# ablab/spades

Measured on NVIDIA H100. Metric: Mk-mers/s (extract+count+index) k=55, 150 bp reads, higher is better.
Workload: dtype u64

## Files before the change

### spades_b200/csrc/count.cu

```cuda
#include <time.h>

#include <algorithm>
#include <chrono>
#include <memory>

#include "sgpu_internal.h"

namespace sg {

__device__ __forceinline__ void prefetch_l2(const void *p) { asm volatile("prefetch.global.L2 [%0];" ::"l"(p)); }

struct ReadsSrc {
    const uint64_t *words;
    const uint64_t *offs;
    const uint32_t *lens;
    int64_t n;
    uint64_t nwords;
    int K;
    static constexpr int kIds = 24;
    static constexpr int kIdLines = 48;
    static constexpr bool kSubRanges = true;
    __device__ __forceinline__ uint64_t first_word(int64_t item) const { return offs[item]; }
    __device__ __forceinline__ uint32_t len(int64_t item) const { return lens[item]; }
    __device__ __forceinline__ void prefetch_items(int64_t item, int lane) const {
// ... 25 lines not shown
        reinterpret_cast<ulonglong2 *>(dst)[1] = make_ulonglong2(k.w[2], k.w[3]);
    } else {
#pragma unroll
        for (int q = 0; q < NW; ++q) dst[q] = k.w[q];
    }
}
template <int NW>
__device__ __forceinline__ Kmer<NW> load_rec(const uint64_t *src) {
    Kmer<NW> k;
    if (NW == 2) {
        ulonglong2 v = *reinterpret_cast<const ulonglong2 *>(src);
        k.w[0] = v.x; k.w[1] = v.y;
    } else if (NW == 4) {
        ulonglong2 a = reinterpret_cast<const ulonglong2 *>(src)[0], b = reinterpret_cast<const ulonglong2 *>(src)[1];
        k.w[0] = a.x; k.w[1] = a.y; k.w[2] = b.x; k.w[3] = b.y;
    } else {
#pragma unroll
        for (int q = 0; q < NW; ++q) k.w[q] = src[q];
    }
    return k;
}

struct LevelA {
    int K;
    uint32_t B;
    uint32_t b_lo, b_hi;
    int rA;
    uint32_t PA;
};

template <int NW>
__device__ __forceinline__ void store_rec_stream(uint64_t *dst, const Kmer<NW> &k) {
    if (NW == 2) {
        asm volatile("st.global.L1::no_allocate.v2.u64 [%0], {%1, %2};" ::"l"(dst), "l"(k.w[0]), "l"(k.w[1]) : "memory");
    } else if (NW == 4) {
        asm volatile("st.global.L1::no_allocate.v2.u64 [%0], {%1, %2};" ::"l"(dst), "l"(k.w[0]), "l"(k.w[1]) : "memory");
        asm volatile("st.global.L1::no_allocate.v2.u64 [%0], {%1, %2};" ::"l"(dst + 2), "l"(k.w[2]), "l"(k.w[3]) : "memory");
    } else {
#pragma unroll
        for (int q = 0; q < NW; ++q) asm volatile("st.global.L1::no_allocate.u64 [%0], %1;" ::"l"(dst + q), "l"(k.w[q]) : "memory");
    }
}

__device__ __forceinline__ int find_item_u(const uint32_t *pref, int nitems, uint32_t i, uint32_t uniform) {
    if (uniform) return (int)(i / uniform);
    int lo = 0, hi = nitems - 1;
    while (lo < hi) {
        int mid = (lo + hi + 1) >> 1;
        if (pref[mid] <= i) lo = mid; else hi = mid - 1;
    }
    return lo;
}

template <int NW>
__device__ __forceinline__ bool part_of(const LevelA &p, const Kmer<NW> &k, uint32_t *part) {
    uint32_t b = kmer_bucket<NW>(k, p.B);
    if (b < p.b_lo || b >= p.b_hi) return false;
    *part = ((b - p.b_lo) << p.rA) | key_top_bits<NW>(k, p.K, p.rA);
    return true;
}

__global__ void levelA_totals_k(const uint32_t *__restrict__ blk_counts, uint32_t PA, int G, uint64_t *__restrict__ part_total) {
    uint32_t part = blockIdx.x * blockDim.x + threadIdx.x;
    if (part >= PA) return;
    uint64_t s = 0;
    for (int g = 0; g < G; ++g) s += blk_counts[(size_t)g * PA + part];
    part_total[part] = s;
}
__global__ void levelA_bases_k(const uint32_t *__restrict__ blk_counts, uint32_t stride, uint32_t PA, int G,
                               const uint64_t *__restrict__ part_start, uint64_t *__restrict__ base) {
    uint32_t part = blockIdx.x * blockDim.x + threadIdx.x;
    if (part >= PA) return;
    uint64_t run = part_start[part];
    for (int g = 0; g < G; ++g) {
        base[(size_t)g * PA + part] = run;
        run += blk_counts[(size_t)g * stride + part];
    }
}

static const int kRollC = 24;
template <bool BOTH> constexpr int kRollWin = BOTH ? kRollC / 2 : kRollC;
static_assert(kRollC <= 33 && kRollC % 8 == 0, "roll_init fetches a chunk's bases from two words; an id row is a whole number of 16-byte words");
static_assert(ReadsSrc::kIds == kRollC && KmerSetSrc::kIds % 8 == 0, "an id row holds a chunk's records");
static const int kRollThreads = 512;

static const int kRollTile = 32;
static const int kRollWarps = kRollThreads / 32;
static const int kRollStageWords = 320;
struct RollWarp {
    uint64_t words[kRollStageWords];
    uint32_t pref[kRollTile + 1];
    uint32_t len[kRollTile];
    uint32_t off[kRollTile];
    uint32_t pad_;
};
static_assert(sizeof(RollWarp) % 8 == 0, "per-warp slices stay 8-byte aligned");
static size_t roll_smem_bytes(uint32_t nslots) { return (((size_t)nslots * 4 + 15) & ~(size_t)15) + (size_t)kRollWarps * sizeof(RollWarp); }
__device__ __forceinline__ RollWarp *roll_warp_slice(unsigned char *raw, uint32_t nslots) {
    return reinterpret_cast<RollWarp *>(raw + (((size_t)nslots * 4 + 15) & ~(size_t)15)) + (threadIdx.x >> 5);
}

template <bool BOTH, class Src>
__device__ __forceinline__ uint32_t roll_warp_setup(const Src &src, int64_t item0, int nitems, RollWarp &rw, uint32_t *uniform, bool *staged) {
    const int lane = threadIdx.x & 31;
    uint32_t c = 0, L = 0;
    uint64_t a = 0, b = 0;
    if (lane < nitems) {
        L = src.len(item0 + lane);
        a = src.first_word(item0 + lane);
        b = a + (((uint64_t)L + 31) >> 5);
        const uint32_t w = (int)L >= src.K ? (uint32_t)((int)L - src.K + 1) : 0u;
        c = (w + kRollWin<BOTH> - 1) / kRollWin<BOTH>;
    }
    uint32_t inc = c;
#pragma unroll
    for (int o = 1; o < 32; o <<= 1) {
        const uint32_t t = __shfl_up_sync(0xffffffffu, inc, o);
        if (lane >= o) inc += t;
    }
    rw.len[lane] = L;
    rw.pref[lane] = inc - c;
    const uint32_t total = __shfl_sync(0xffffffffu, inc, 31);
    if (lane == 31) rw.pref[kRollTile] = total;
    const uint32_t c0 = __shfl_sync(0xffffffffu, c, 0);
    const bool same = __all_sync(0xffffffffu, lane >= nitems || c == c0);
    *uniform = (same && c0) ? c0 : 0u;
    const uint64_t w0 = __shfl_sync(0xffffffffu, a, 0);
    const bool ok = lane >= nitems || (a >= w0 && b >= a && b - w0 <= (uint64_t)kRollStageWords);
    const bool st = __all_sync(0xffffffffu, ok);
    if (st) {
        rw.off[lane] = (uint32_t)(a - w0);
        uint32_t end = lane < nitems ? (uint32_t)(b - w0) : 0u;
#pragma unroll
        for (int o = 16; o; o >>= 1) end = max(end, __shfl_xor_sync(0xffffffffu, end, o));
        uint64_t tmp[kRollStageWords / 32];
#pragma unroll
        for (int j = 0; j < kRollStageWords / 32; ++j) tmp[j] = (uint32_t)(lane + 32 * j) < end ? __ldg(src.words + w0 + lane + 32 * j) : 0ull;
#pragma unroll
        for (int j = 0; j < kRollStageWords / 32; ++j) if ((uint32_t)(lane + 32 * j) < end) rw.words[lane + 32 * j] = tmp[j];
    }
    *staged = st;
    __syncwarp();
    return total;
}

template <bool BOTH, class Src>
__global__ void roll_tile_ids_k(Src src, int64_t ntiles, uint32_t *__restrict__ out) {
    const int64_t t = (int64_t)blockIdx.x * (blockDim.x >> 5) + (threadIdx.x >> 5);
    if (t >= ntiles) return;
    const int lane = threadIdx.x & 31;
    const int64_t item = t * kRollTile + lane;
    uint32_t s = 0;
    if (item < src.n) {
        const int L = (int)src.len(item);
        const uint32_t w = L >= src.K ? (uint32_t)(L - src.K + 1) : 0u;
        s = (w + kRollWin<BOTH> - 1) / kRollWin<BOTH>;
    }
    for (int o = 16; o; o >>= 1) s += __shfl_down_sync(0xffffffffu, s, o);
    if (lane == 0) out[t] = s * Src::kIds;
}

struct RollUnit { int it, j0, cnt; };
template <bool BOTH>
__device__ __forceinline__ RollUnit roll_unit(const RollWarp &rw, int nitems, uint32_t u, uint32_t unif, int K) {
    constexpr int C = kRollWin<BOTH>;
    RollUnit q;
    q.it = find_item_u(rw.pref, nitems, u, unif);
    q.j0 = (int)(u - rw.pref[q.it]) * C;
    const int nwin = (int)rw.len[q.it] - K + 1;
    q.cnt = nwin - q.j0 < C ? nwin - q.j0 : C;
    return q;
}

template <int NW, class Src, bool BOTH>
__global__ void __launch_bounds__(kRollThreads, 2) levelA_count_roll_k(Src src, LevelA p, uint32_t *__restrict__ blk_counts,
                                                                      const uint64_t *__restrict__ tile_off, uint16_t *__restrict__ ids) {
    extern __shared__ __align__(16) unsigned char sm_raw[];
    uint32_t *hist = reinterpret_cast<uint32_t *>(sm_raw);
    RollWarp &rw = *roll_warp_slice(sm_raw, p.PA);
    for (uint32_t i = threadIdx.x; i < p.PA; i += blockDim.x) hist[i] = 0;
    __syncthreads();
    const int K = p.K;
    const int lane = threadIdx.x & 31, warp = threadIdx.x >> 5;
    const int64_t ntiles = (src.n + kRollTile - 1) / kRollTile;
    const int64_t per = (ntiles + gridDim.x - 1) / gridDim.x;
    const int64_t t0 = (int64_t)blockIdx.x * per, t1 = min(ntiles, t0 + per);
    for (int64_t t = t0 + warp; t < t1; t += kRollWarps) {
        const int64_t item0 = t * kRollTile;
        const int nitems = (int)min((int64_t)kRollTile, src.n - item0);
        uint32_t unif = 0;
        bool staged = false;
        const bool has_next = t + kRollWarps < t1;
        const int64_t nx = (t + kRollWarps) * kRollTile;
        uint64_t next_w0 = 0;
        if (has_next) {
            next_w0 = src.first_word(nx);
            src.prefetch_items(nx, lane);
        }
        const uint32_t nunits = roll_warp_setup<BOTH>(src, item0, nitems, rw, &unif, &staged);
        uint64_t *row = ids ? reinterpret_cast<uint64_t *>(ids + tile_off[t]) : nullptr;
        for (uint32_t u = lane; u < nunits; u += 32) {
            const RollUnit q = roll_unit<BOTH>(rw, nitems, u, unif, K);
            const uint64_t *seq = staged ? static_cast<const uint64_t *>(rw.words + rw.off[q.it]) : src.words + src.first_word(item0 + q.it);
            RollState<NW> st;
            roll_init<NW>(st, seq, q.j0, K, q.cnt);
            const int nrec = BOTH ? 2 * q.cnt : q.cnt;
#pragma unroll 1
            for (int g = 0; g < Src::kIds / 4; ++g) {
                uint64_t acc = 0;
#pragma unroll
                for (int e = 0; e < 4; ++e) {
                    const int s = 4 * g + e;
                    uint32_t id = 0xffffu;
                    if (s < nrec) {
                        if (s > 0 && !(BOTH && (e & 1))) roll_next<NW>(st, K);
                        const Kmer<NW> k = BOTH ? ((e & 1) ? st.r : st.f) : kmer_is_minimal<NW>(st.f, st.r) ? st.f : st.r;
                        uint32_t part;
                        if (part_of<NW>(p, k, &part)) { atomicAdd(&hist[part], 1u); id = part; }
                    }
                    acc |= (uint64_t)id << (16 * e);
                }
                if (row) row[(size_t)u * (Src::kIds / 4) + g] = acc;
            }
        }
        if (has_next && lane < 10 && next_w0 + 16 * lane < src.nwords) prefetch_l2(src.words + next_w0 + 16 * lane);
        __syncwarp();
    }
    __syncthreads();
    uint32_t *out = blk_counts + (size_t)blockIdx.x * p.PA;
    for (uint32_t i = threadIdx.x; i < p.PA; i += blockDim.x) out[i] += hist[i];
}

static const uint32_t kABatchMin = 1024;
static_assert(kABatchMin / kRollWarps >= 32 * 2, "a warp's share of the smallest batch holds one window of a warp step");
__host__ __device__ __forceinline__ size_t abatch_offset(uint32_t PA) {
    return ((((size_t)2 * PA * 4 + 15) & ~(size_t)15) + (size_t)kRollWarps * sizeof(RollWarp) + 15) & ~(size_t)15;
}
template <int NW, bool PLANNED>
constexpr size_t abatch_rec_bytes() { return NW * sizeof(uint64_t) + (PLANNED ? sizeof(uint16_t) : sizeof(uint32_t) + sizeof(uint16_t)); }

static const uint32_t kABatchNoTag = 0xffffffffu;
static const int kABatchPartBits = 13;
template <int NW, class Src, bool BOTH>
__global__ void __launch_bounds__(kRollThreads, 2) levelA_scatter_roll_k(Src src, LevelA p, uint64_t *__restrict__ base, uint64_t *__restrict__ out,
                                                                        uint32_t row_stride, uint32_t cap) {
    extern __shared__ __align__(16) unsigned char sm_raw[];
    __shared__ uint32_t s_fill;
    __shared__ uint32_t warp_tot[kRollWarps];
    const uint32_t PA = p.PA;
    uint32_t *cur = reinterpret_cast<uint32_t *>(sm_raw);
    uint32_t *cnt = cur + PA;
    RollWarp &rw = *roll_warp_slice(sm_raw, 2 * PA);
    uint64_t *stage = reinterpret_cast<uint64_t *>(sm_raw + abatch_offset(PA));
    uint32_t *tags = reinterpret_cast<uint32_t *>(stage + (size_t)cap * NW);
    uint16_t *idx = reinterpret_cast<uint16_t *>(tags + cap);
    uint64_t *mybase = base + (size_t)blockIdx.x * row_stride;
    const uint64_t region0 = mybase[0];
    for (uint32_t i = threadIdx.x; i < PA; i += blockDim.x) { cur[i] = (uint32_t)(mybase[i] - region0); cnt[i] = 0; }
    if (threadIdx.x == 0) s_fill = 0;
    __syncthreads();
    uint64_t *const out0 = out + region0 * NW;
    const int K = p.K;
    const int lane = threadIdx.x & 31, warp = threadIdx.x >> 5;
    const uint32_t lt_mask = (1u << lane) - 1u;
    const int64_t ntiles = (src.n + kRollTile - 1) / kRollTile;
    const int64_t per = (ntiles + gridDim.x - 1) / gridDim.x;
    const int64_t t0 = (int64_t)blockIdx.x * per, t1 = min(ntiles, t0 + per);

    int64_t t = t0 + warp;
    bool need_setup = true;
    int nitems = 0;
    uint32_t nunits = 0, unif = 0;
    bool staged = false;
    uint64_t next_w0 = 0;
    int u = 0, s = 0, cnt_w = 0;
    RollState<NW> st;
    for (;;) {
        while (t < t1) {
            if (need_setup) {
                const int64_t item0 = t * kRollTile;
                nitems = (int)min((int64_t)kRollTile, src.n - item0);
                const int64_t nx = (t + kRollWarps) * kRollTile;
                if (t + kRollWarps < t1) {
                    next_w0 = src.first_word(nx);
                    src.prefetch_items(nx, lane);
                }
                nunits = roll_warp_setup<BOTH>(src, item0, nitems, rw, &unif, &staged);
                u = lane - 32; s = cnt_w = 0;
                need_setup = false;
            }
            if (s >= cnt_w && u < (int)nunits) {
                u += 32;
                if (u < (int)nunits) {
                    const RollUnit q = roll_unit<BOTH>(rw, nitems, (uint32_t)u, unif, K);
                    const uint64_t *seq = staged ? static_cast<const uint64_t *>(rw.words + rw.off[q.it]) : src.words + src.first_word(t * kRollTile + q.it);
                    roll_init<NW>(st, seq, q.j0, K, q.cnt);
                    s = 0; cnt_w = BOTH ? 2 * q.cnt : q.cnt;
                }
            }
            const bool act = s < cnt_w;
            if (!__any_sync(0xffffffffu, act)) {
                if (t + kRollWarps < t1 && lane < 10 && next_w0 + 16 * lane < src.nwords) prefetch_l2(src.words + next_w0 + 16 * lane);
                __syncwarp();
                t += kRollWarps;
                need_setup = true;
                continue;
            }
            uint32_t part = 0;
            bool mine = false;
            Kmer<NW> k;
            if (act) {
                const bool fwd = BOTH ? !(s & 1) : kmer_is_minimal<NW>(st.f, st.r);
#pragma unroll
                for (int j = 0; j < NW; ++j) k.w[j] = fwd ? st.f.w[j] : st.r.w[j];
                mine = part_of<NW>(p, k, &part);
            }
            const uint32_t bal = __ballot_sync(0xffffffffu, mine);
            if (bal) {
                const uint32_t n = __popc(bal);
                uint32_t b0 = 0;
                if (lane == 0) b0 = atomicAdd(&s_fill, n);
                b0 = __shfl_sync(0xffffffffu, b0, 0);
                if (b0 + n > cap) {
                    if (b0 < cap && (uint32_t)lane < cap - b0) tags[b0 + lane] = kABatchNoTag;
                    break;
                }
                if (mine) {
                    const uint32_t i = b0 + __popc(bal & lt_mask);
                    const uint32_t rank = atomicAdd(&cnt[part], 1u) & 0xffffu;
                    store_rec<NW>(stage + (size_t)i * NW, k);
                    tags[i] = (rank << kABatchPartBits) | part;
                }
            }
            if (act && ++s < cnt_w && (!BOTH || !(s & 1))) roll_next<NW>(st, K);
        }
        const bool more = __syncthreads_or(t < t1);
        const uint32_t nslots = min(s_fill, cap);
        const uint32_t own = (PA + kRollThreads - 1) / kRollThreads;
        const uint32_t j0 = min(PA, threadIdx.x * own), j1 = min(PA, j0 + own);
        uint32_t sum = 0;
        for (uint32_t j = j0; j < j1; ++j) sum += cnt[j] & 0xffffu;
        uint32_t inc = sum;
#pragma unroll
        for (int o = 1; o < 32; o <<= 1) {
            const uint32_t v = __shfl_up_sync(0xffffffffu, inc, o);
            if (lane >= o) inc += v;
        }
        if (lane == 31) warp_tot[warp] = inc;
        __syncthreads();
        uint32_t wb = 0, total = 0;
#pragma unroll
        for (int w = 0; w < kRollWarps; ++w) { const uint32_t v = warp_tot[w]; if (w < warp) wb += v; total += v; }
        uint32_t o = wb + inc - sum;
        for (uint32_t j = j0; j < j1; ++j) {
            const uint32_t c = cnt[j] & 0xffffu;
            o += c;
            cnt[j] = o << 16;
            cur[j] += c;
        }
        if (threadIdx.x == 0) s_fill = 0;
        __syncthreads();
        for (uint32_t i = threadIdx.x; i < nslots; i += kRollThreads) {
            const uint32_t tg = tags[i];
            if (tg == kABatchNoTag) continue;
            idx[(cnt[tg & ((1u << kABatchPartBits) - 1)] >> 16) - 1 - (tg >> kABatchPartBits)] = (uint16_t)i;
        }
        __syncthreads();
        for (uint32_t q = threadIdx.x; q < total; q += kRollThreads) {
            const uint32_t i = idx[q], tg = tags[i];
            const uint32_t slot = cur[tg & ((1u << kABatchPartBits) - 1)] - 1 - (tg >> kABatchPartBits);
            store_rec_stream<NW>(out0 + (size_t)slot * NW, load_rec<NW>(stage + (size_t)i * NW));
        }
        __syncthreads();
        if (!more) break;
    }
    for (uint32_t i = threadIdx.x; i < PA; i += blockDim.x) mybase[i] = region0 + cur[i];
}

template <int NW, class Src, bool BOTH>
__global__ void __launch_bounds__(kRollThreads, 2) levelA_scatter_plan_k(Src src, LevelA p, uint64_t *__restrict__ base, uint64_t *__restrict__ out,
                                                                        const uint64_t *__restrict__ tile_off, const uint16_t *__restrict__ ids,
                                                                        uint32_t id_lo, uint32_t row_stride, uint32_t q_lo, uint64_t ids_len, uint32_t cap) {
    extern __shared__ __align__(16) unsigned char sm_raw[];
    __shared__ uint32_t warp_tot[kRollWarps];
    constexpr int kR = BOTH ? 2 : 1;
    constexpr int kRowV = Src::kIds / 8;
    const uint32_t PA = p.PA;
    uint32_t *cur = reinterpret_cast<uint32_t *>(sm_raw);
    uint32_t *run = cur + PA;
    RollWarp &rw = *roll_warp_slice(sm_raw, 2 * PA);
    uint64_t *stage = reinterpret_cast<uint64_t *>(sm_raw + abatch_offset(PA));
    uint16_t *ptag = reinterpret_cast<uint16_t *>(stage + (size_t)cap * NW);
    uint64_t *mybase = base + (size_t)blockIdx.x * row_stride + q_lo;
    const uint64_t region0 = mybase[0];
    for (uint32_t i = threadIdx.x; i < PA; i += blockDim.x) { cur[i] = (uint32_t)(mybase[i] - region0); run[i] = 0; }
    __syncthreads();
    uint64_t *const out0 = out + region0 * NW;
    const int K = p.K;
    const int lane = threadIdx.x & 31, warp = threadIdx.x >> 5;
    const int64_t ntiles = (src.n + kRollTile - 1) / kRollTile;
    const int64_t per = (ntiles + gridDim.x - 1) / gridDim.x;
    const int64_t t0 = (int64_t)blockIdx.x * per, t1 = min(ntiles, t0 + per);
    const uint32_t share = cap / kRollWarps;

    int64_t pt = t0 + warp;
    int pj = 0, ps = 0;
    uint32_t pn = 0;
    bool p_enter = true;
    const ulonglong2 *prow = nullptr;
    int64_t rt = pt;
    int rj = 0, rs = 0;
    bool need_setup = true;
    int nitems = 0;
    uint32_t nunits = 0, unif = 0;
    bool staged = false;
    uint64_t next_w0 = 0;
    const ulonglong2 *row = nullptr;
    for (;;) {
        uint32_t room = share;
        while (pt < t1) {
            if (p_enter) {
                const uint64_t a = tile_off[pt], b = tile_off[pt + 1];
                if (pt + kRollWarps < t1) {
                    const uint64_t nr = tile_off[pt + kRollWarps];
                    if ((Src::kIdLines >= 32 || lane < Src::kIdLines) && nr + 64 * lane < ids_len) prefetch_l2(ids + nr + 64 * lane);
                    if (lane < Src::kIdLines - 32 && nr + 64 * (32 + lane) < ids_len) prefetch_l2(ids + nr + 64 * (32 + lane));
                }
                pn = (uint32_t)((b - a) / Src::kIds);
                prow = reinterpret_cast<const ulonglong2 *>(ids + a);
                p_enter = false;
            }
            if ((uint32_t)pj * 32 >= pn) {
                pt += kRollWarps; pj = 0; ps = 0; p_enter = true;
                continue;
            }
            if (room < 32 * kR) break;
            const uint32_t u = (uint32_t)pj * 32 + lane;
            uint64_t idq[Src::kIds / 4];
#pragma unroll
            for (int v = 0; v < kRowV; ++v) {
                ulonglong2 x = make_ulonglong2(~0ull, ~0ull);
                if (u < pn) x = __ldg(prow + (size_t)u * kRowV + v);
                idq[2 * v] = x.x; idq[2 * v + 1] = x.y;
            }
            int end = Src::kIds;
#pragma unroll
            for (int e = 0; e < Src::kIds; e += kR) {
                uint32_t part[kR];
                bool own[kR];
                uint32_t c = 0;
#pragma unroll
                for (int r = 0; r < kR; ++r) {
                    part[r] = (uint32_t)((idq[(e + r) / 4] >> (16 * ((e + r) % 4))) & 0xffffu) - id_lo;
                    own[r] = e >= ps && part[r] < PA;
                    c += __popc(__ballot_sync(0xffffffffu, own[r]));
                }
                if (c > room) { end = e; break; }
                room -= c;
#pragma unroll
                for (int r = 0; r < kR; ++r) if (own[r]) atomicAdd(&run[part[r]], 1u);
            }
            if (end < Src::kIds) { ps = end; break; }
            ++pj; ps = 0;
        }
        const bool more = __syncthreads_or(pt < t1);
        const uint32_t own = (PA + kRollThreads - 1) / kRollThreads;
        const uint32_t j0 = min(PA, threadIdx.x * own), j1 = min(PA, j0 + own);
        uint32_t sum = 0;
        for (uint32_t j = j0; j < j1; ++j) sum += run[j] & 0xffffu;
        uint32_t inc = sum;
#pragma unroll
        for (int o = 1; o < 32; o <<= 1) {
            const uint32_t v = __shfl_up_sync(0xffffffffu, inc, o);
            if (lane >= o) inc += v;
        }
        if (lane == 31) warp_tot[warp] = inc;
        __syncthreads();
        uint32_t wb = 0, total = 0;
#pragma unroll
        for (int w = 0; w < kRollWarps; ++w) { const uint32_t v = warp_tot[w]; if (w < warp) wb += v; total += v; }
        uint32_t o = wb + inc - sum;
        for (uint32_t j = j0; j < j1; ++j) {
            const uint32_t c = run[j] & 0xffffu;
            run[j] = o << 16;
            o += c;
            cur[j] += c;
        }
        __syncthreads();
        while (rt < pt || (rt == pt && (rj < pj || (rj == pj && rs < ps)))) {
            if (need_setup) {
                const int64_t item0 = rt * kRollTile;
                nitems = (int)min((int64_t)kRollTile, src.n - item0);
                const int64_t nx = (rt + kRollWarps) * kRollTile;
                if (rt + kRollWarps < t1) {
                    next_w0 = src.first_word(nx);
                    src.prefetch_items(nx, lane);
                }
                nunits = roll_warp_setup<BOTH>(src, item0, nitems, rw, &unif, &staged);
                row = reinterpret_cast<const ulonglong2 *>(ids + tile_off[rt]);
                need_setup = false;
            }
            if ((uint32_t)rj * 32 >= nunits) {
                if (rt + kRollWarps < t1 && lane < 10 && next_w0 + 16 * lane < src.nwords) prefetch_l2(src.words + next_w0 + 16 * lane);
                __syncwarp();
                rt += kRollWarps; rj = 0; rs = 0;
                need_setup = true;
                continue;
            }
            const int end = (rt == pt && rj == pj) ? ps : Src::kIds;
            const int u = rj * 32 + lane;
            if (u < (int)nunits) {
                const RollUnit q = roll_unit<BOTH>(rw, nitems, (uint32_t)u, unif, K);
                const int s_end = min(end, BOTH ? 2 * q.cnt : q.cnt);
                if (rs < s_end) {
                    uint64_t idq[Src::kIds / 4];
#pragma unroll
                    for (int v = 0; v < kRowV; ++v) {
                        const ulonglong2 x = __ldg(row + (size_t)u * kRowV + v);
                        idq[2 * v] = x.x; idq[2 * v + 1] = x.y;
                    }
                    for (int w = 0; w < rs / 4; ++w) {
#pragma unroll
                        for (int v = 0; v + 1 < Src::kIds / 4; ++v) idq[v] = idq[v + 1];
                    }
                    idq[0] >>= 16 * (rs & 3);
                    const uint64_t *seq = staged ? static_cast<const uint64_t *>(rw.words + rw.off[q.it]) : src.words + src.first_word(rt * kRollTile + q.it);
                    RollState<NW> st;
                    roll_init<NW>(st, seq, q.j0 + rs / kR, K, q.cnt - rs / kR);
                    for (int s = rs;;) {
                        const uint32_t part = (uint32_t)(idq[0] & 0xffffu) - id_lo;
                        if (part < PA) {
                            const bool fwd = BOTH ? !(s & 1) : kmer_is_minimal<NW>(st.f, st.r);
                            Kmer<NW> k;
#pragma unroll
                            for (int j = 0; j < NW; ++j) k.w[j] = fwd ? st.f.w[j] : st.r.w[j];
                            const uint32_t pos = atomicAdd(&run[part], 1u << 16) >> 16;
                            store_rec<NW>(stage + (size_t)pos * NW, k);
                            ptag[pos] = (uint16_t)part;
                        }
                        if (++s >= s_end) break;
                        if (!BOTH || !(s & 1)) roll_next<NW>(st, K);
                        if ((s & 3) == 0) {
#pragma unroll
                            for (int v = 0; v + 1 < Src::kIds / 4; ++v) idq[v] = idq[v + 1];
                        } else {
                            idq[0] >>= 16;
                        }
                    }
                }
            }
            if (end == Src::kIds) { ++rj; rs = 0; } else rs = end;
        }
        __syncthreads();
        for (uint32_t q = threadIdx.x; q < total; q += kRollThreads) {
            const uint32_t part = ptag[q];
            const uint32_t slot = cur[part] - (run[part] >> 16) + q;
            store_rec_stream<NW>(out0 + (size_t)slot * NW, load_rec<NW>(stage + (size_t)q * NW));
        }
        if (!more) break;
    }
    for (uint32_t i = threadIdx.x; i < PA; i += blockDim.x) mybase[i] = region0 + cur[i];
}

struct Seg {
    uint64_t start;
    uint64_t len;
    uint32_t bits;
    uint32_t bb;
};

__global__ void seg_init_k(const uint64_t *__restrict__ part_start, const uint64_t *__restrict__ part_total, uint32_t PA, int rA,
                           uint32_t b_lo, Seg *__restrict__ segs) {
    uint32_t part = blockIdx.x * blockDim.x + threadIdx.x;
    if (part >= PA) return;
    Seg s;
    s.start = part_start[part]; s.len = part_total[part]; s.bits = (uint32_t)rA; s.bb = ((b_lo + (part >> rA)) << 1) | 0u;
    segs[part] = s;
}

struct Pieces {
    const uint64_t *pbase;
    const uint32_t *cnt;
    uint32_t cnt_stride, PA;
    int G;
};
static const int kMaxPieces = 1024;

__global__ void stage_rows_k(const uint32_t *__restrict__ cnt, uint32_t cnt_stride, uint32_t PA, uint64_t *__restrict__ rel, uint64_t *__restrict__ row_total) {
    __shared__ uint64_t wsum[8];
    __shared__ uint64_t carry_s;
    const uint32_t *row = cnt + (size_t)blockIdx.x * cnt_stride;
    uint64_t *out = rel + (size_t)blockIdx.x * PA;
    const int lane = threadIdx.x & 31, warp = threadIdx.x >> 5;
    if (threadIdx.x == 0) carry_s = 0;
    __syncthreads();
    for (uint32_t b = 0; b < PA; b += blockDim.x) {
        const uint32_t i = b + threadIdx.x;
        const uint64_t v = i < PA ? row[i] : 0;
        uint64_t inc = v;
#pragma unroll
        for (int o = 1; o < 32; o <<= 1) {
            uint64_t t = __shfl_up_sync(0xffffffffu, inc, o);
            if (lane >= o) inc += t;
        }
        if (lane == 31) wsum[warp] = inc;
        __syncthreads();
        uint64_t wb = 0, all = 0;
        for (int w = 0; w < 8; ++w) { if (w < warp) wb += wsum[w]; all += wsum[w]; }
        const uint64_t carry = carry_s;
        if (i < PA) out[i] = carry + wb + inc - v;
        __syncthreads();
        if (threadIdx.x == 0) carry_s = carry + all;
        __syncthreads();
    }
    if (threadIdx.x == 0) row_total[blockIdx.x] = carry_s;
}
__global__ void stage_add_k(uint64_t *__restrict__ rel, const uint64_t *__restrict__ row_start, uint32_t PA, int G) {
    const uint64_t i = (uint64_t)blockIdx.x * blockDim.x + threadIdx.x;
    if (i >= (uint64_t)G * PA) return;
    rel[i] += row_start[i / PA];
}

struct RefinePlan { uint32_t cap, target, rmax; int total_bits; };
__device__ __forceinline__ int plan_r(const RefinePlan &rp, uint64_t len, uint32_t bits) {
    if (len <= rp.cap) return 0;
    int rem = rp.total_bits - (int)bits;
    if (rem <= 0) return 0;
    uint64_t want = (len + rp.target - 1) / rp.target;
    int r = 1;
    while (r < (int)rp.rmax && (1ull << r) < want) ++r;
    return r < rem ? r : rem;
}
__global__ void refine_plan_k(const Seg *__restrict__ segs, uint64_t n, RefinePlan rp, uint32_t *__restrict__ nchild, uint32_t *__restrict__ isw, int force_all) {
    uint64_t i = (uint64_t)blockIdx.x * blockDim.x + threadIdx.x;
    if (i >= n) return;
    int r = plan_r(rp, segs[i].len, segs[i].bits);
    nchild[i] = r ? (1u << r) : 1u;
    isw[i] = (r || force_all) ? 1u : 0u;
}
__global__ void refine_copy_k(const Seg *__restrict__ segs, uint64_t n, const uint32_t *__restrict__ isw, const uint64_t *__restrict__ child_base,
                              const uint64_t *__restrict__ work_pos, Seg *__restrict__ nsegs, uint64_t *__restrict__ worklist) {
    uint64_t i = (uint64_t)blockIdx.x * blockDim.x + threadIdx.x;
    if (i >= n) return;
    if (isw[i]) worklist[work_pos[i]] = i;
    else nsegs[child_base[i]] = segs[i];
}

static const int kRThreads = 1024;
static const int kRWarps = kRThreads / 32;
static const int kRMaxBins = 2048;
template <int NW> struct RBatch {
    static const int RPT = NW == 1 ? 12 : NW == 2 ? 8 : NW == 3 ? 4 : 3;
    static const int N = RPT * kRThreads;
    static constexpr size_t smem() { return (size_t)N * (NW * sizeof(uint64_t) + sizeof(uint32_t)); }
};

template <int NW, bool PIECED>
__global__ void __launch_bounds__(kRThreads) refine_k(const Seg *__restrict__ segs, const uint64_t *__restrict__ worklist, uint64_t nwork,
                                                     const uint64_t *__restrict__ child_base, RefinePlan rp, int K,
                                                     uint64_t *__restrict__ buf0, uint64_t *__restrict__ buf1, Seg *__restrict__ nsegs,
                                                     unsigned long long *__restrict__ work_counter, Pieces pc) {
    constexpr int RPT = RBatch<NW>::RPT, N = RBatch<NW>::N;
    __shared__ uint32_t hist[kRMaxBins];
    __shared__ uint32_t run_off[kRMaxBins];
    __shared__ uint32_t run_slot[kRMaxBins];
    __shared__ uint32_t warp_tot[kRWarps];
    __shared__ unsigned long long s_w;
    __shared__ uint64_t pc_start[PIECED ? kMaxPieces : 1];
    __shared__ uint32_t pc_len[PIECED ? kMaxPieces : 1];
    extern __shared__ uint64_t sm_refine_dyn[];
    uint64_t *stage = sm_refine_dyn;
    uint32_t *stage_slot = reinterpret_cast<uint32_t *>(stage + (size_t)N * NW);
    const int lane = threadIdx.x & 31, warp = threadIdx.x >> 5;
    for (;;) {
        if (threadIdx.x == 0) s_w = atomicAdd(work_counter, 1ull);
        __syncthreads();
        const uint64_t wi = s_w;
        __syncthreads();
        if (wi >= nwork) return;
        const uint64_t si = worklist[wi];
        const Seg s = segs[si];
        const int r = plan_r(rp, s.len, s.bits);
        const uint32_t nb = 1u << r;
        const uint64_t *src = ((s.bb & 1) ? buf1 : buf0) + s.start * NW;
        uint64_t *dst = ((s.bb & 1) ? buf0 : buf1) + s.start * NW;
        if (PIECED) {
            for (int g = threadIdx.x; g < pc.G; g += blockDim.x) {
                pc_start[g] = pc.pbase[(size_t)g * pc.PA + si];
                pc_len[g] = pc.cnt[(size_t)g * pc.cnt_stride + si];
            }
        }
        for (uint32_t i = threadIdx.x; i < nb; i += blockDim.x) hist[i] = 0;
        __syncthreads();
        if (PIECED) {
            for (int g = warp; g < pc.G; g += kRWarps) {
                const uint64_t *ps = buf0 + pc_start[g] * NW;
                const uint32_t n = pc_len[g];
                uint32_t i = lane;
                for (; i + 96 < n; i += 128) {
                    const Kmer<NW> k0 = load_rec<NW>(ps + (uint64_t)i * NW), k1 = load_rec<NW>(ps + (uint64_t)(i + 32) * NW);
                    const Kmer<NW> k2 = load_rec<NW>(ps + (uint64_t)(i + 64) * NW), k3 = load_rec<NW>(ps + (uint64_t)(i + 96) * NW);
                    atomicAdd(&hist[key_bits<NW>(k0, K, (int)s.bits, r)], 1u);
                    atomicAdd(&hist[key_bits<NW>(k1, K, (int)s.bits, r)], 1u);
                    atomicAdd(&hist[key_bits<NW>(k2, K, (int)s.bits, r)], 1u);
                    atomicAdd(&hist[key_bits<NW>(k3, K, (int)s.bits, r)], 1u);
                }
                for (; i < n; i += 32) {
                    const Kmer<NW> k = load_rec<NW>(ps + (uint64_t)i * NW);
                    atomicAdd(&hist[key_bits<NW>(k, K, (int)s.bits, r)], 1u);
                }
            }
        } else {
            for (uint64_t i = threadIdx.x; i < s.len; i += blockDim.x) {
                Kmer<NW> k = load_rec<NW>(src + i * NW);
                atomicAdd(&hist[key_bits<NW>(k, K, (int)s.bits, r)], 1u);
            }
        }
        __syncthreads();
        uint32_t a = 0, b = 0;
        const uint32_t i0 = 2 * threadIdx.x;
        if (i0 < nb) { a = hist[i0]; hist[i0] = 0; }
        if (i0 + 1 < nb) { b = hist[i0 + 1]; hist[i0 + 1] = 0; }
        uint32_t v = a + b, inc = v;
#pragma unroll
        for (int o = 1; o < 32; o <<= 1) {
            uint32_t t = __shfl_up_sync(0xffffffffu, inc, o);
            if (lane >= o) inc += t;
        }
        if (lane == 31) warp_tot[warp] = inc;
        __syncthreads();
        if (warp == 0) {
            uint32_t w = warp_tot[lane], winc = w;
#pragma unroll
            for (int o = 1; o < 32; o <<= 1) {
                uint32_t t = __shfl_up_sync(0xffffffffu, winc, o);
                if (lane >= o) winc += t;
            }
            warp_tot[lane] = winc - w;
        }
        __syncthreads();
        const uint32_t ex = warp_tot[warp] + inc - v;
        const uint64_t cb = child_base[si];
        if (i0 < nb) {
            Seg c; c.start = s.start + ex; c.len = a; c.bits = s.bits + (uint32_t)r; c.bb = s.bb ^ 1u;
            nsegs[cb + i0] = c;
        }
        if (i0 + 1 < nb) {
            Seg c; c.start = s.start + ex + a; c.len = b; c.bits = s.bits + (uint32_t)r; c.bb = s.bb ^ 1u;
            nsegs[cb + i0 + 1] = c;
        }
        uint32_t cur0 = ex, cur1 = ex + a;

        Kmer<NW> rec[RPT];
        uint32_t have = 0;
        int pg = warp;
        uint32_t ppos = 0;
        uint64_t cpos = 0;
        auto load_batch = [&]() {
            have = 0;
            if (PIECED) {
                while (pg < pc.G && ppos >= pc_len[pg]) { pg += kRWarps; ppos = 0; }
                if (pg < pc.G) {
                    const uint64_t *ps = buf0 + pc_start[pg] * NW;
                    const uint32_t n = pc_len[pg];
#pragma unroll
                    for (int j = 0; j < RPT; ++j) {
                        const uint32_t i = ppos + lane + 32 * j;
                        if (i < n) { rec[j] = load_rec<NW>(ps + (uint64_t)i * NW); have |= 1u << j; }
                    }
                    ppos += 32 * RPT;
                }
            } else {
#pragma unroll
                for (int j = 0; j < RPT; ++j) {
                    const uint64_t i = cpos + threadIdx.x + (uint64_t)kRThreads * j;
                    if (i < s.len) { rec[j] = load_rec<NW>(src + i * NW); have |= 1u << j; }
                }
                cpos += N;
            }
        };
        load_batch();
        for (;;) {
            uint32_t tag[RPT];
#pragma unroll
            for (int j = 0; j < RPT; ++j) {
                if (have >> j & 1u) {
                    const uint32_t bin = key_bits<NW>(rec[j], K, (int)s.bits, r);
                    tag[j] = (atomicAdd(&hist[bin], 1u) << 11) | bin;
                }
            }
            if (!__syncthreads_or(have)) break;
            const uint32_t c0 = i0 < nb ? hist[i0] : 0u, c1 = i0 + 1 < nb ? hist[i0 + 1] : 0u;
            const uint32_t bv = c0 + c1;
            uint32_t binc = bv;
#pragma unroll
            for (int o = 1; o < 32; o <<= 1) {
                uint32_t t = __shfl_up_sync(0xffffffffu, binc, o);
                if (lane >= o) binc += t;
            }
            if (lane == 31) warp_tot[warp] = binc;
            __syncthreads();
            uint32_t w = warp_tot[lane], winc = w;
#pragma unroll
            for (int o = 1; o < 32; o <<= 1) {
                uint32_t t = __shfl_up_sync(0xffffffffu, winc, o);
                if (lane >= o) winc += t;
            }
            const uint32_t total = __shfl_sync(0xffffffffu, winc, 31);
            const uint32_t off = __shfl_sync(0xffffffffu, winc - w, warp) + binc - bv;
            if (i0 < nb) { run_off[i0] = off; run_slot[i0] = cur0; hist[i0] = 0; cur0 += c0; }
            if (i0 + 1 < nb) { run_off[i0 + 1] = off + c0; run_slot[i0 + 1] = cur1; hist[i0 + 1] = 0; cur1 += c1; }
            __syncthreads();
#pragma unroll
            for (int j = 0; j < RPT; ++j) {
                if (have >> j & 1u) {
                    const uint32_t bin = tag[j] & (kRMaxBins - 1), rank = tag[j] >> 11;
                    const uint32_t p = run_off[bin] + rank;
                    store_rec<NW>(stage + (size_t)p * NW, rec[j]);
                    stage_slot[p] = run_slot[bin] + rank;
                }
            }
            load_batch();
            __syncthreads();
            for (uint32_t p = threadIdx.x; p < total; p += kRThreads)
                store_rec_stream<NW>(dst + (uint64_t)stage_slot[p] * NW, load_rec<NW>(stage + (size_t)p * NW));
        }
    }
}

template <int NW> struct SortCfg { static const int CAP = NW <= 2 ? 2048 : 1024; };
static const int kSThreads = 512;
static const int kSWarps = kSThreads / 32;

template <int NW>
__device__ __forceinline__ void lsd_pass(const uint64_t *A, uint64_t *Bf, uint32_t n, int K, int pos, int width, uint32_t *cnt ,
                                         uint32_t *tot ) {
    static_assert(kSThreads >= 256, "one thread per digit");
    const int lane = threadIdx.x & 31, warp = threadIdx.x >> 5;
    const uint32_t chunk = ((n + kSWarps * 32 - 1) / (kSWarps * 32)) * 32;
    const uint32_t w0 = warp * chunk;
    for (int i = threadIdx.x; i < kSWarps * 256; i += kSThreads) cnt[i] = 0;
    __syncthreads();
    for (uint32_t r = 0; r < chunk; r += 32) {
        const uint32_t i = w0 + r + lane;
        uint32_t d = 256;
// ... 493 lines not shown
        nsegs = tot[0];
    }
    ctx->times.refine_rounds_max = std::max(ctx->times.refine_rounds_max, rounds);
    ctx->times.refine += tm.stop();
    DArr<uint32_t> ndist(ctx, nsegs + 1);
    DArr<unsigned long long> stats(ctx, 4);
    SG_CUDA(cudaMemsetAsync(ndist.p, 0, ndist.bytes(), st));
    SG_CUDA(cudaMemsetAsync(stats.p, 0, 32, st));
    SG_CUDA(cudaMemsetAsync(wcounter.p, 0, 8, st));
    tm.start();
    {
        auto launch = [&](auto kernel, size_t smem) {
            SG_CUDA(cudaFuncSetAttribute(kernel, cudaFuncAttributeMaxDynamicSharedMemorySize, (int)smem));
            int occ = 1;
            SG_CUDA(cudaOccupancyMaxActiveBlocksPerMultiprocessor(&occ, kernel, kSThreads, smem));
            if (occ < 1) occ = 1;
            int grid = (int)std::min<uint64_t>(nsegs, (uint64_t)ctx->num_sms * occ);
            if (grid < 1) grid = 1;
            kernel<<<grid, kSThreads, smem, st>>>(segs.p, nsegs, K, X.p, Y.p, ndist.p, wcounter.p, stats.p);
        };
        launch(local_sort3_k<NW, kSortBinBits, CAP>, SortSmem<NW, kSortBinBits, CAP>::bytes);
        ctx->launches++;
        SG_CUDA(cudaGetLastError());
    }
    DArr<uint64_t> dbase(ctx, nsegs + 1);
    exclusive_scan_u32_to_u64(ctx, ndist.p, dbase.p, nsegs + 1);
    uint64_t D = 0;
    unsigned long long h_stats[4];
    SG_CUDA(cudaMemcpyAsync(&D, dbase.p + nsegs, 8, cudaMemcpyDeviceToHost, st));
    SG_CUDA(cudaMemcpyAsync(h_stats, stats.p, 32, cudaMemcpyDeviceToHost, st));
    SG_CUDA(cudaStreamSynchronize(st));
    ctx->times.local_sort += tm.stop();
    tr.mark("local sort");
    SG_CHECK(h_stats[0] == 0, 6, "internal: oversize segment with unfixed key bits reached the local sort");
    ctx->times.sort_lsd_fallbacks += h_stats[1];
    ctx->times.sort_oversize_equal += h_stats[2];
    if (sink) sink->drain();
    Chunk ch;
    ch.n = (int64_t)D; ch.b_lo = (int)b_lo; ch.b_hi = b_hi; ch.first = first;
    ch.keys.alloc(ctx, (size_t)D * NW + 2, true);
    if (want_counts) ch.counts.alloc(ctx, (size_t)D + 1, true);
    tm.start();
    if (nsegs) {
        compact_k<NW><<<div_up((int64_t)nsegs * 32, 256), 256, 0, st>>>(segs.p, nsegs, ndist.p, dbase.p, X.p, Y.p, K, want_counts ? 1 : 0,
                                                                     double_selfrc ? 1 : 0, ch.keys.p, ch.counts.p, d_bsz_p);
        ctx->launches++;
        SG_CUDA(cudaGetLastError());
    }
    ctx->times.compact += tm.stop();
    tr.mark("compact");
    ch_out = std::move(ch);
}

template <int NW, class Src, bool BOTH>
struct LevelAJob {
    Ctx *ctx = nullptr;
    std::vector<Src> srcs;
    int K = 0, B = 0, rA = 0, G = 0;
    int s_lo = 0, s_hi = 0;
    uint32_t PA_all = 0;
    bool use_ids = false;
    DArr<uint32_t> blk_counts;
    DArr<uint64_t> part_total_all;
    std::vector<DArr<uint64_t>> tile_off;
    std::vector<DArr<uint16_t>> ids;
    std::vector<uint64_t> h_part;
    ChunkStager *stage = nullptr;
    template <class F>
    void for_each_src(F &&launch) const {
        for (size_t si = 0; si < srcs.size(); ++si) {
            Src src = srcs[si];
            if (stage) stage->acquire(si, &src.words, nullptr);
            if (src.n) launch(si, src);
            if (stage) stage->release(si);
        }
    }
    uint64_t bucket_records(int b) const {
        uint64_t s = 0;
        for (uint32_t q = 0; q < (1u << rA); ++q) s += h_part[((size_t)(b - s_lo) << rA) + q];
        return s;
    }
};

static int levelA_ctas_per_sm() { return 2; }
template <int NW, bool PLANNED>
static size_t levelA_batch_smem(uint32_t PA, uint32_t *cap) {
    static_assert(kLevelAMaxParts <= (1 << kABatchPartBits) && kLevelAMaxParts <= 0xffff, "a batch tag holds the partition");
    int dev = 0, per_sm = 0, per_cta = 0, reserved = 0;
    SG_CUDA(cudaGetDevice(&dev));
    SG_CUDA(cudaDeviceGetAttribute(&per_sm, cudaDevAttrMaxSharedMemoryPerMultiprocessor, dev));
    SG_CUDA(cudaDeviceGetAttribute(&per_cta, cudaDevAttrMaxSharedMemoryPerBlockOptin, dev));
    SG_CUDA(cudaDeviceGetAttribute(&reserved, cudaDevAttrReservedSharedMemoryPerBlock, dev));
    const size_t rec = abatch_rec_bytes<NW, PLANNED>(), fixed = abatch_offset(PA), kStatic = 128;
    size_t room = (size_t)per_sm / levelA_ctas_per_sm() - (size_t)reserved - kStatic;
    if (room < fixed + kABatchMin * rec) room = (size_t)per_cta - kStatic;
    SG_CHECK(room >= fixed + kABatchMin * rec, 6, "internal: level-A batch does not fit shared memory");
    *cap = (uint32_t)std::min<size_t>((room - fixed) / rec, 32768) & ~31u;
    SG_CHECK(!PLANNED || *cap / kRollWarps >= 32 * 2, 6, "internal: level-A warp share below one window step");
    return fixed + (size_t)*cap * rec;
}
static int levelA_key_bits(uint64_t est_records, int B, int total_bits, uint32_t target, uint32_t pa_max) {
    const int want = ilog2_floor(est_records / target + 1) + 1;
    const int bbits = ilog2_floor((uint64_t)B) + (((1u << ilog2_floor((uint64_t)B)) < (uint32_t)B) ? 1 : 0);
    int rA = want - bbits;
    if (rA < 0) rA = 0;
    while (rA > 0 && ((uint64_t)B << rA) > pa_max) --rA;
    if (rA > total_bits) rA = total_bits;
    if (rA > 13) rA = 13;
    return rA;
}

template <int NW, class Src, bool BOTH>
static void levelA_count(LevelAJob<NW, Src, BOTH> &job, Timer &tm, Trace &tr) {
    Ctx *ctx = job.ctx;
    cudaStream_t st = ctx->stream;
    const uint32_t PA_all = job.PA_all;
    const int G = job.G;
    SG_CHECK(PA_all >= 1 && PA_all <= (uint32_t)kLevelAMaxParts, 6, "internal: level-A partition table too large");
    LevelA pa_all;
    pa_all.K = job.K; pa_all.B = (uint32_t)job.B; pa_all.b_lo = (uint32_t)job.s_lo; pa_all.b_hi = (uint32_t)job.s_hi; pa_all.rA = job.rA; pa_all.PA = PA_all;
    job.blk_counts.alloc(ctx, (size_t)G * PA_all);
    job.part_total_all.alloc(ctx, (size_t)PA_all + 1);
    job.h_part.assign(PA_all, 0);
    SG_CUDA(cudaMemsetAsync(job.blk_counts.p, 0, job.blk_counts.bytes(), st));
    job.tile_off.clear(); job.ids.clear();
    job.tile_off.resize(job.srcs.size()); job.ids.resize(job.srcs.size());
    const double free0 = (double)ctx->free_bytes();
    std::vector<uint64_t> nslots(job.srcs.size(), 0);
    uint64_t all_slots = 0;
    for (size_t si = 0; si < job.srcs.size(); ++si) {
        const Src &src = job.srcs[si];
        if (src.n == 0) continue;
        const int64_t ntiles = (src.n + kRollTile - 1) / kRollTile;
        DArr<uint32_t> ttot(ctx, (size_t)ntiles + 1);
        job.tile_off[si].alloc(ctx, (size_t)ntiles + 1);
        SG_CUDA(cudaMemsetAsync(ttot.p + ntiles, 0, 4, st));
        roll_tile_ids_k<BOTH><<<div_up(ntiles, 8), 256, 0, st>>>(src, ntiles, ttot.p);
        ctx->launches++;
        exclusive_scan_u32_to_u64(ctx, ttot.p, job.tile_off[si].p, (size_t)ntiles + 1);
        SG_CUDA(cudaMemcpyAsync(&nslots[si], job.tile_off[si].p + ntiles, 8, cudaMemcpyDeviceToHost, st));
        SG_CUDA(cudaStreamSynchronize(st));
        all_slots += nslots[si];
    }
    job.use_ids = PA_all < 0xffffu && (double)all_slots * 2.0 < free0 * 0.20;
    for (size_t si = 0; si < job.srcs.size(); ++si) {
        if (!job.use_ids) job.tile_off[si] = DArr<uint64_t>();
        else if (job.srcs[si].n) job.ids[si].alloc(ctx, (size_t)nslots[si] + 8);
    }
    tm.start();
    SG_CUDA(cudaFuncSetAttribute(levelA_count_roll_k<NW, Src, BOTH>, cudaFuncAttributeMaxDynamicSharedMemorySize, (int)roll_smem_bytes(PA_all)));
    job.for_each_src([&](size_t si, const Src &src) {
        levelA_count_roll_k<NW, Src, BOTH><<<G, kRollThreads, roll_smem_bytes(PA_all), st>>>(src, pa_all, job.blk_counts.p, job.tile_off[si].p, job.ids[si].p);
        ctx->launches++;
    });
    SG_CUDA(cudaGetLastError());
    levelA_totals_k<<<div_up(PA_all, 256), 256, 0, st>>>(job.blk_counts.p, PA_all, G, job.part_total_all.p);
    ctx->launches++;
    SG_CUDA(cudaMemcpyAsync(job.h_part.data(), job.part_total_all.p, (size_t)PA_all * 8, cudaMemcpyDeviceToHost, st));
    SG_CUDA(cudaStreamSynchronize(st));
    ctx->times.extract_count += tm.stop();
    tr.mark("A1 count+totals");
}

template <int NW, class Src, bool BOTH>
static void levelA_scatter(LevelAJob<NW, Src, BOTH> &job, int b_lo, int b_hi, uint64_t I_pass, uint64_t total_records, uint64_t *X, uint64_t *pbase_buf,
                           Pieces &pcs, Timer &tm, Trace &tr) {
    Ctx *ctx = job.ctx;
    cudaStream_t st = ctx->stream;
    const int G = job.G;
    const uint32_t PA_all = job.PA_all;
    const uint32_t p_lo = (uint32_t)(b_lo - job.s_lo) << job.rA;
    LevelA pa;
    pa.K = job.K; pa.B = (uint32_t)job.B; pa.b_lo = (uint32_t)b_lo; pa.b_hi = (uint32_t)b_hi; pa.rA = job.rA; pa.PA = (uint32_t)(b_hi - b_lo) << job.rA;
    const uint32_t PA = pa.PA;
    SG_CHECK(PA >= 1 && PA <= (uint32_t)kLevelAMaxParts && G <= kMaxPieces, 6, "internal: level-A pass geometry");
    DArr<uint64_t> base(ctx, (size_t)G * PA);
    {
        DArr<uint64_t> row_total(ctx, (size_t)G + 1), row_start(ctx, (size_t)G + 1);
        SG_CUDA(cudaMemsetAsync(row_total.p + G, 0, 8, st));
        stage_rows_k<<<G, 256, 0, st>>>(job.blk_counts.p + p_lo, PA_all, PA, base.p, row_total.p);
        exclusive_scan_u64(ctx, row_total.p, row_start.p, (size_t)G + 1);
        stage_add_k<<<div_up((int64_t)G * PA, 256), 256, 0, st>>>(base.p, row_start.p, PA, G);
        ctx->launches += 2;
        SG_CUDA(cudaMemcpyAsync(pbase_buf, base.p, (size_t)G * PA * 8, cudaMemcpyDeviceToDevice, st));
    }
    pcs.pbase = pbase_buf; pcs.cnt = job.blk_counts.p + p_lo; pcs.cnt_stride = PA_all; pcs.PA = PA; pcs.G = G;
    tm.start();
    int nsub_auto = (int)(4.0 * (double)I_pass / (double)std::max<uint64_t>(1, total_records) + 0.5);
    nsub_auto = std::min(4, std::max(1, nsub_auto));
    uint32_t nsub = job.use_ids && !BOTH && Src::kSubRanges ? (uint32_t)(tuning().a_sub ? tuning().a_sub : nsub_auto) : 1u;
    if (nsub > PA) nsub = PA;
    for (uint32_t sb = 0; sb < nsub; ++sb) {
        const uint32_t q_lo = (uint32_t)((uint64_t)PA * sb / nsub), q_hi = (uint32_t)((uint64_t)PA * (sb + 1) / nsub);
        if (q_hi == q_lo) continue;
        LevelA pa_sub = pa;
        pa_sub.PA = q_hi - q_lo;
        uint32_t cap = 0;
        const size_t smem = job.use_ids ? levelA_batch_smem<NW, true>(pa_sub.PA, &cap) : levelA_batch_smem<NW, false>(pa_sub.PA, &cap);
        if (job.use_ids) SG_CUDA(cudaFuncSetAttribute(levelA_scatter_plan_k<NW, Src, BOTH>, cudaFuncAttributeMaxDynamicSharedMemorySize, (int)smem));
        else SG_CUDA(cudaFuncSetAttribute(levelA_scatter_roll_k<NW, Src, BOTH>, cudaFuncAttributeMaxDynamicSharedMemorySize, (int)smem));
        job.for_each_src([&](size_t si, const Src &src) {
            if (job.use_ids)
                levelA_scatter_plan_k<NW, Src, BOTH><<<G, kRollThreads, smem, st>>>(src, pa_sub, base.p, X, job.tile_off[si].p, job.ids[si].p, p_lo + q_lo, PA, q_lo, (uint64_t)job.ids[si].n, cap);
            else
                levelA_scatter_roll_k<NW, Src, BOTH><<<G, kRollThreads, smem, st>>>(src, pa, base.p, X, PA, cap);
            ctx->launches++; ctx->times.level_a_scatters++;
        });
    }
    SG_CUDA(cudaGetLastError());
    ctx->times.extract_scatter += tm.stop();
    tr.mark("A2 scatter");
}

static double pass_bytes_needed(uint64_t recs, size_t W) { return (double)recs * W * 2.0 + (double)recs * (W + 4) * 0.6 + (64 << 20); }

template <int NW, bool BOTH, class Src>
static void run_count(Ctx *ctx, const std::vector<Src> &srcs, int K, int B, bool want_counts, bool double_selfrc, uint64_t est_records, KSet *out,
                      ResultSink *sink = nullptr, ChunkStager *stage = nullptr) {
    const int total_bits = 2 * K;
    const size_t W = 8 * NW;
    cudaStream_t st = ctx->stream;
    Timer tm(st);
    Trace tr(st);

    out->bsz.assign(B, 0);
    DArr<unsigned long long> d_bsz(ctx, B);
    SG_CUDA(cudaMemsetAsync(d_bsz.p, 0, B * sizeof(unsigned long long), st));

    const int rA = levelA_key_bits(est_records, B, total_bits, sort_target<NW>(), tuning().pa_max);
    ctx->times.level_a_key_bits = (uint64_t)rA;
    const int SR = std::max(1, kLevelAMaxParts >> rA);
    const int n_ranges = (B + SR - 1) / SR;
    int64_t first = 0;
    for (int s_lo = 0; s_lo < B; s_lo += SR) {
        const int share = (kMaxChunks - (int)out->chunks.size()) / (n_ranges - s_lo / SR);
        LevelAJob<NW, Src, BOTH> job;
        job.ctx = ctx; job.srcs = srcs; job.K = K; job.B = B; job.rA = rA; job.G = ctx->num_sms * levelA_ctas_per_sm(); job.stage = stage;
        job.s_lo = s_lo; job.s_hi = std::min(B, s_lo + SR);
        job.PA_all = (uint32_t)(job.s_hi - job.s_lo) << rA;
        levelA_count(job, tm, tr);
        auto current_limit = [&]() {
            return ctx->hbm_budget ? (ctx->hbm_budget > ctx->allocated ? ctx->hbm_budget - ctx->allocated : 0) : (size_t)(ctx->free_bytes() * 0.90);
        };
        uint64_t total_records = 0;
        for (int b = job.s_lo; b < job.s_hi; ++b) total_records += job.bucket_records(b);
        uint64_t pass_target = total_records;
        bool capped = false;
        {
            double lim_sim = (double)current_limit(), inflight = 0;
            int npass_sim = 0, b = job.s_lo;
            while (b < job.s_hi) {
                uint64_t I = 0; const int b0 = b;
                while (b < job.s_hi) {
                    const uint64_t ib = job.bucket_records(b);
                    if (b > b0 && pass_bytes_needed(I + ib, W) + inflight > lim_sim) break;
                    I += ib; ++b;
                }
                if (sink) inflight = (double)I * (W + 4) * 0.5;
// ... 610 lines not shown
```

Before: 8719.

## Use 1024-thread single-CTA level-A kernels, fast-path planned scatter, split gather pieces

```diff
diff --git a/spades_b200/csrc/count.cu b/spades_b200/csrc/count.cu
--- a/spades_b200/csrc/count.cu
+++ b/spades_b200/csrc/count.cu
@@ -131,10 +131,11 @@
 template <bool BOTH> constexpr int kRollWin = BOTH ? kRollC / 2 : kRollC;
 static_assert(kRollC <= 33 && kRollC % 8 == 0, "roll_init fetches a chunk's bases from two words; an id row is a whole number of 16-byte words");
 static_assert(ReadsSrc::kIds == kRollC && KmerSetSrc::kIds % 8 == 0, "an id row holds a chunk's records");
-static const int kRollThreads = 512;
+static const int kRollThreads = 1024;
 
 static const int kRollTile = 32;
 static const int kRollWarps = kRollThreads / 32;
+static_assert(kRollWarps == 32, "the scatter kernels' claim reads one warp total per lane");
 static const int kRollStageWords = 320;
 struct RollWarp {
     uint64_t words[kRollStageWords];
@@ -222,7 +223,7 @@
 }
 
 template <int NW, class Src, bool BOTH>
-__global__ void __launch_bounds__(kRollThreads, 2) levelA_count_roll_k(Src src, LevelA p, uint32_t *__restrict__ blk_counts,
+__global__ void __launch_bounds__(kRollThreads, 1) levelA_count_roll_k(Src src, LevelA p, uint32_t *__restrict__ blk_counts,
                                                                       const uint64_t *__restrict__ tile_off, uint16_t *__restrict__ ids) {
     extern __shared__ __align__(16) unsigned char sm_raw[];
     uint32_t *hist = reinterpret_cast<uint32_t *>(sm_raw);
@@ -281,7 +282,6 @@
 }
 
 static const uint32_t kABatchMin = 1024;
-static_assert(kABatchMin / kRollWarps >= 32 * 2, "a warp's share of the smallest batch holds one window of a warp step");
 __host__ __device__ __forceinline__ size_t abatch_offset(uint32_t PA) {
     return ((((size_t)2 * PA * 4 + 15) & ~(size_t)15) + (size_t)kRollWarps * sizeof(RollWarp) + 15) & ~(size_t)15;
 }
@@ -291,7 +291,7 @@
 static const uint32_t kABatchNoTag = 0xffffffffu;
 static const int kABatchPartBits = 13;
 template <int NW, class Src, bool BOTH>
-__global__ void __launch_bounds__(kRollThreads, 2) levelA_scatter_roll_k(Src src, LevelA p, uint64_t *__restrict__ base, uint64_t *__restrict__ out,
+__global__ void __launch_bounds__(kRollThreads, 1) levelA_scatter_roll_k(Src src, LevelA p, uint64_t *__restrict__ base, uint64_t *__restrict__ out,
                                                                         uint32_t row_stride, uint32_t cap) {
     extern __shared__ __align__(16) unsigned char sm_raw[];
     __shared__ uint32_t s_fill;
@@ -397,9 +397,8 @@
         }
         if (lane == 31) warp_tot[warp] = inc;
         __syncthreads();
-        uint32_t wb = 0, total = 0;
-#pragma unroll
-        for (int w = 0; w < kRollWarps; ++w) { const uint32_t v = warp_tot[w]; if (w < warp) wb += v; total += v; }
+        const uint32_t wt = warp_tot[lane];
+        const uint32_t wb = __reduce_add_sync(0xffffffffu, lane < warp ? wt : 0u), total = __reduce_add_sync(0xffffffffu, wt);
         uint32_t o = wb + inc - sum;
         for (uint32_t j = j0; j < j1; ++j) {
             const uint32_t c = cnt[j] & 0xffffu;
@@ -427,7 +426,7 @@
 }
 
 template <int NW, class Src, bool BOTH>
-__global__ void __launch_bounds__(kRollThreads, 2) levelA_scatter_plan_k(Src src, LevelA p, uint64_t *__restrict__ base, uint64_t *__restrict__ out,
+__global__ void __launch_bounds__(kRollThreads, 1) levelA_scatter_plan_k(Src src, LevelA p, uint64_t *__restrict__ base, uint64_t *__restrict__ out,
                                                                         const uint64_t *__restrict__ tile_off, const uint16_t *__restrict__ ids,
                                                                         uint32_t id_lo, uint32_t row_stride, uint32_t q_lo, uint64_t ids_len, uint32_t cap) {
     extern __shared__ __align__(16) unsigned char sm_raw[];
@@ -492,6 +491,21 @@
                 if (u < pn) x = __ldg(prow + (size_t)u * kRowV + v);
                 idq[2 * v] = x.x; idq[2 * v + 1] = x.y;
             }
+            uint32_t nown = 0;
+#pragma unroll
+            for (int e = 0; e < Src::kIds; ++e)
+                nown += (e >= ps && (uint32_t)((idq[e / 4] >> (16 * (e % 4))) & 0xffffu) - id_lo < PA) ? 1u : 0u;
+            const uint32_t cstep = NW <= 2 ? __reduce_add_sync(0xffffffffu, nown) : ~0u;
+            if (cstep <= room) {
+                room -= cstep;
+#pragma unroll
+                for (int e = 0; e < Src::kIds; ++e) {
+                    const uint32_t part = (uint32_t)((idq[e / 4] >> (16 * (e % 4))) & 0xffffu) - id_lo;
+                    if (e >= ps && part < PA) atomicAdd(&run[part], 1u);
+                }
+                ++pj; ps = 0;
+                continue;
+            }
             int end = Src::kIds;
 #pragma unroll
             for (int e = 0; e < Src::kIds; e += kR) {
@@ -525,9 +539,8 @@
         }
         if (lane == 31) warp_tot[warp] = inc;
         __syncthreads();
-        uint32_t wb = 0, total = 0;
-#pragma unroll
-        for (int w = 0; w < kRollWarps; ++w) { const uint32_t v = warp_tot[w]; if (w < warp) wb += v; total += v; }
+        const uint32_t wt = warp_tot[lane];
+        const uint32_t wb = __reduce_add_sync(0xffffffffu, lane < warp ? wt : 0u), total = __reduce_add_sync(0xffffffffu, wt);
         uint32_t o = wb + inc - sum;
         for (uint32_t j = j0; j < j1; ++j) {
             const uint32_t c = run[j] & 0xffffu;
@@ -634,6 +647,7 @@
     int G;
 };
 static const int kMaxPieces = 1024;
+static const int kGatherSplit = 4;
 
 __global__ void stage_rows_k(const uint32_t *__restrict__ cnt, uint32_t cnt_stride, uint32_t PA, uint64_t *__restrict__ rel, uint64_t *__restrict__ row_total) {
     __shared__ uint64_t wsum[8];
@@ -733,16 +747,20 @@
         const uint32_t nb = 1u << r;
         const uint64_t *src = ((s.bb & 1) ? buf1 : buf0) + s.start * NW;
         uint64_t *dst = ((s.bb & 1) ? buf0 : buf1) + s.start * NW;
+        const int np = PIECED ? kGatherSplit * pc.G : 0;
         if (PIECED) {
-            for (int g = threadIdx.x; g < pc.G; g += blockDim.x) {
-                pc_start[g] = pc.pbase[(size_t)g * pc.PA + si];
-                pc_len[g] = pc.cnt[(size_t)g * pc.cnt_stride + si];
+            for (int v = threadIdx.x; v < np; v += blockDim.x) {
+                const int g = v / kGatherSplit, h = v % kGatherSplit;
+                const uint32_t n = pc.cnt[(size_t)g * pc.cnt_stride + si];
+                const uint32_t a = (uint32_t)((uint64_t)n * h / kGatherSplit), b = (uint32_t)((uint64_t)n * (h + 1) / kGatherSplit);
+                pc_start[v] = pc.pbase[(size_t)g * pc.PA + si] + a;
+                pc_len[v] = b - a;
             }
         }
         for (uint32_t i = threadIdx.x; i < nb; i += blockDim.x) hist[i] = 0;
         __syncthreads();
         if (PIECED) {
-            for (int g = warp; g < pc.G; g += kRWarps) {
+            for (int g = warp; g < np; g += kRWarps) {
                 const uint64_t *ps = buf0 + pc_start[g] * NW;
                 const uint32_t n = pc_len[g];
                 uint32_t i = lane;
@@ -808,8 +826,8 @@
         auto load_batch = [&]() {
             have = 0;
             if (PIECED) {
-                while (pg < pc.G && ppos >= pc_len[pg]) { pg += kRWarps; ppos = 0; }
-                if (pg < pc.G) {
+                while (pg < np && ppos >= pc_len[pg]) { pg += kRWarps; ppos = 0; }
+                if (pg < np) {
                     const uint64_t *ps = buf0 + pc_start[pg] * NW;
                     const uint32_t n = pc_len[pg];
 #pragma unroll
@@ -1469,7 +1487,7 @@
     }
 };
 
-static int levelA_ctas_per_sm() { return 2; }
+static int levelA_ctas_per_sm() { return 1; }
 template <int NW, bool PLANNED>
 static size_t levelA_batch_smem(uint32_t PA, uint32_t *cap) {
     static_assert(kLevelAMaxParts <= (1 << kABatchPartBits) && kLevelAMaxParts <= 0xffff, "a batch tag holds the partition");
@@ -1478,9 +1496,8 @@
     SG_CUDA(cudaDeviceGetAttribute(&per_sm, cudaDevAttrMaxSharedMemoryPerMultiprocessor, dev));
     SG_CUDA(cudaDeviceGetAttribute(&per_cta, cudaDevAttrMaxSharedMemoryPerBlockOptin, dev));
     SG_CUDA(cudaDeviceGetAttribute(&reserved, cudaDevAttrReservedSharedMemoryPerBlock, dev));
-    const size_t rec = abatch_rec_bytes<NW, PLANNED>(), fixed = abatch_offset(PA), kStatic = 128;
-    size_t room = (size_t)per_sm / levelA_ctas_per_sm() - (size_t)reserved - kStatic;
-    if (room < fixed + kABatchMin * rec) room = (size_t)per_cta - kStatic;
+    const size_t rec = abatch_rec_bytes<NW, PLANNED>(), fixed = abatch_offset(PA), kStatic = 256;
+    const size_t room = std::min<size_t>((size_t)per_sm - (size_t)reserved, (size_t)per_cta) - kStatic;
     SG_CHECK(room >= fixed + kABatchMin * rec, 6, "internal: level-A batch does not fit shared memory");
     *cap = (uint32_t)std::min<size_t>((room - fixed) / rec, 32768) & ~31u;
     SG_CHECK(!PLANNED || *cap / kRollWarps >= 32 * 2, 6, "internal: level-A warp share below one window step");
@@ -1560,7 +1577,7 @@
     LevelA pa;
     pa.K = job.K; pa.B = (uint32_t)job.B; pa.b_lo = (uint32_t)b_lo; pa.b_hi = (uint32_t)b_hi; pa.rA = job.rA; pa.PA = (uint32_t)(b_hi - b_lo) << job.rA;
     const uint32_t PA = pa.PA;
-    SG_CHECK(PA >= 1 && PA <= (uint32_t)kLevelAMaxParts && G <= kMaxPieces, 6, "internal: level-A pass geometry");
+    SG_CHECK(PA >= 1 && PA <= (uint32_t)kLevelAMaxParts && kGatherSplit * G <= kMaxPieces, 6, "internal: level-A pass geometry");
     DArr<uint64_t> base(ctx, (size_t)G * PA);
     {
         DArr<uint64_t> row_total(ctx, (size_t)G + 1), row_start(ctx, (size_t)G + 1);
```

After: 8921 (median of 6 runs). 1.02x the previous value.
